# DerekRowell/AudioSDR

Hardware: AMD Instinct MI355X
Metric: Msamples/s through full SSB demod chain, batched 128-sample blocks (higher is better)
Workload: dtype f32

## Files before the change

### audiosdr_amd/csrc/asdr_kernels.hip

```cpp
#include <hip/hip_runtime.h>
#include <stdint.h>
#include <stddef.h>
#include <string.h>
#include <stdlib.h>
#include <type_traits>

#include "asdr_device.h"
#include "asdr_tables.h"
#include "../../include/asdr.h"

#define W0 0
#define W1 128
#define PH 256
#define XP 0
#ifndef ASDR_STRIDE
#define ASDR_STRIDE 388
#endif
#ifndef ASDR_AGC_QUIET_PATH
#define ASDR_AGC_QUIET_PATH 1
#endif
#ifndef ASDR_MW_OWN_STORES
#define ASDR_MW_OWN_STORES 1
#endif
#ifndef ASDR_AGC_LEAN
#define ASDR_AGC_LEAN 1
#endif
#ifndef ASDR_MW_AGC_PIPELINED
#define ASDR_MW_AGC_PIPELINED 0
#endif
#ifndef ASDR_ONEBLK
#define ASDR_ONEBLK 1
#endif
#ifndef ASDR_MW
#define ASDR_MW 1
#endif
#ifndef ASDR_MW_SHARE
#define ASDR_MW_SHARE 7
#endif
#ifndef ASDR_MIX_KEEP_Q
#define ASDR_MIX_KEEP_Q 1
#endif
#ifndef ASDR_UNIT_SCALE
#define ASDR_UNIT_SCALE 1
#endif
#ifndef ASDR_C16
#define ASDR_C16 0
#endif
#ifndef ASDR_C16_MIN_WAVES
#define ASDR_C16_MIN_WAVES 64
#endif
#ifndef ASDR_MW_MIN_WAVES
#define ASDR_MW_MIN_WAVES 64
#endif
#ifndef ASDR_MW_PRIO
#define ASDR_MW_PRIO 2
#endif
#ifndef ASDR_CHAIN_PRIO
#define ASDR_CHAIN_PRIO 0
#endif
#define CHAIN_PRIO_ON() do { if (ASDR_CHAIN_PRIO) __builtin_amdgcn_s_setprio(ASDR_CHAIN_PRIO); } while (0)
#define CHAIN_PRIO_OFF() do { if (ASDR_CHAIN_PRIO) __builtin_amdgcn_s_setprio(0); } while (0)
// ... 839 lines not shown
  constexpr bool DO1 = (ROLE == 0 || ROLE == 1 || PRE_ROLE || ROLE == 6 || ROLE == 7), DO2 = (ROLE == 0 || ROLE == 2 || POST_ROLE || ROLE == 6 || ROLE == 7),
                 DO3 = (ROLE == 0 || ROLE == 3 || POST_ROLE || ROLE == 6 || ROLE == 7);
  constexpr bool TO_ALS = (ROLE == 6 || ROLE == 7 || ROLE == 10);
#ifndef ASDR_ALS_FULL_OPT
#define ASDR_ALS_FULL_OPT 2
#endif
  constexpr bool ALS_LOOPFREE = (ASDR_ONEBLK_ALS != 0) && (ONEBLK_ || (ROLE >= 4 && !LOOPED_ROLE && ASDR_ONEBLK_ROLES));
  constexpr bool ALS_FULL_OPT = (ASDR_ALS_FULL_OPT >= 1) && ASDR_COMPACT_ROWS(STRIDE) && ALS_LOOPFREE,
                 ALS_FULL_OPT2 = (ASDR_ALS_FULL_OPT >= 2) && ASDR_COMPACT_ROWS(STRIDE) && ALS_LOOPFREE;
  constexpr bool STREAM = (ROLE >= 1 && ROLE <= 3);
  constexpr bool PIPE_PK = ((ASDR_PIPE_PK_MASK & 1) && HAS_ALS) || ((ASDR_PIPE_PK_MASK & 2) && !HAS_ALS && !HAS_SAM && ROLE == 0) ||
                           ((ASDR_PIPE_PK_MASK & 4) && (HAS_SAM || ROLE > 3)) || ((ASDR_PIPE_PK_MASK & 8) && STREAM);
  if (ROLE == 0 && a.run_if != nullptr && *a.run_if == 0u) return;
  constexpr bool MW = (WAVES > 1) && !HAS_SAM && (ROLE == 0);
  constexpr int MW_SHARE = MW ? ASDR_MW_SHARE : 0;
  const int wave = (WAVES > 1) ? (int)(threadIdx.x >> 6) : 0;
#ifndef ASDR_MW_ROT
#define ASDR_MW_ROT 0
#endif
  const uint32_t mw_b = blockIdx.x;
  const uint32_t mw_rot = (ASDR_MW_ROT == 0) ? mw_b : (ASDR_MW_ROT == 1) ? (mw_b >> 3) : (ASDR_MW_ROT == 2) ? ((mw_b >> 3) + (mw_b >> 8)) :
                          (ASDR_MW_ROT == 3) ? ((mw_b * 0x9E3779B1u) >> 30) : (ASDR_MW_ROT == 4) ? ((mw_b >> 3) % 3u) : (mw_b >> 5);
  const int mw_rel = MW ? (int)(((uint32_t)wave - mw_rot) & (uint32_t)(WAVES - 1)) : 0;
  float *const mwx = lds_wg + WAVES * 8 * STRIDE;
#ifndef ASDR_MW_STRAGGLER_PRIO
#define ASDR_MW_STRAGGLER_PRIO 0
#endif
  int *const mw_prog = reinterpret_cast<int *>(lds_wg + WAVES * 8 * STRIDE + 8 * WAVES * 16 + 260);
  int *const mw_flags = mw_prog + 4;
  constexpr bool PIPE_AGC = MW && WAVES == 4 && (MW_SHARE & 7) == 7 && (ASDR_MW_AGC_PIPELINED != 0) && (ASDR_AGC_LEAN != 0) && (ASDR_MW_OWN_STORES != 0) && ABL_ON(ABL_AGC) && ABL_ON(ABL_AF) && ABL_ON(ABL_NB);
  if constexpr (PIPE_AGC) { if (threadIdx.x < 3) mw_flags[1 + threadIdx.x] = 0; }
  if constexpr (MW && ASDR_MW_STRAGGLER_PRIO != 0) { if ((threadIdx.x & 63) == 0) mw_prog[wave] = 0; }
  auto mw_straggler = [&](int point) {
    if constexpr (MW && ASDR_MW_STRAGGLER_PRIO != 0) {
      if ((threadIdx.x & 63) == 0) mw_prog[wave] = point;
      const int4 pr = *reinterpret_cast<const int4 *>(mw_prog);
      const int behind = (pr.x < point) + (pr.y < point) + (pr.z < point) + (pr.w < point);
      const bool last = __builtin_amdgcn_readfirstlane(behind) == 0;
      if (last) __builtin_amdgcn_s_setprio(ASDR_MW_STRAGGLER_PRIO); else __builtin_amdgcn_s_setprio(0);
    }
  };
  constexpr int MWX = 16;
  auto mw_channel = [&](int q) -> int { const int sidx = (int)blockIdx.x * (8 * WAVES) + q; return (sidx < a.n_sched) ? a.direct_ch0 + sidx : a.n_channels; };
  const int wave_g = STREAM ? (int)blockIdx.x % a.stream_waves : (int)blockIdx.x * WAVES + wave;
  float *const lds = lds_wg + wave * 8 * STRIDE;
  const int lane = threadIdx.x & 63, c8 = lane >> 3, s8_ = lane & 7;
#ifndef ASDR_MW_SINE_LDS
#define ASDR_MW_SINE_LDS 0
#endif
  constexpr bool MW_SINE = MW && (ASDR_MW_SINE_LDS != 0);
  constexpr bool MW_SINE_LAZY = MW_SINE && (ASDR_MW_SINE_LDS == 2) && (MW_SHARE & 2) != 0 && WAVES == 4;
  constexpr bool SINE_LDS = HAS_SAM || (MW_SINE && !MW_SINE_LAZY);
  constexpr bool SINE_LDS_PC = HAS_SAM || MW_SINE;
  float *const sine_tab = HAS_SAM ? lds_wg + WAVES * 8 * STRIDE : (MW_SINE ? lds_wg + WAVES * 8 * STRIDE + 8 * WAVES * 16 : nullptr);
  float *const sine = SINE_LDS ? sine_tab : nullptr;
  int *const mw_sflag = reinterpret_cast<int *>(lds_wg + WAVES * 8 * STRIDE + 8 * WAVES * 16 + 260) + 8;
  if (HAS_SAM) for (int i = lane; i < ASDR_SINE_TABLE_LEN; i += 64) sine_tab[i] = c_sine[i];
  if (MW_SINE && !MW_SINE_LAZY) { for (int i = (int)threadIdx.x; i < ASDR_SINE_TABLE_LEN; i += 64 * WAVES) sine_tab[i] = c_sine[i]; __syncthreads(); }

  int4 slot = make_int4(a.n_channels, 0, 0, 0);
  const bool mw_pad = MW && (wave_g * 8 >= a.n_sched);
  if (UNIFORM && a.direct_ch0 >= 0) slot = make_int4(mw_pad ? a.n_channels : a.direct_ch0 + wave_g * 8 + c8, (int)a.direct_mode, (int)a.direct_flags, (int)((a.direct_lo & 0xFFu) | (wave_g == 0 ? a.lo_writer_bit : 0u)));
  else if (WAVES == 1 || wave_g * 8 < a.n_sched) slot = *reinterpret_cast<const int4 *>(a.sched + wave_g * 8 + c8);
  else { const ChanParams *pd = a.params + a.n_channels; slot.y = (int)pd->mode; slot.z = (int)pd->flags; }
  const int ch_ = slot.x;
  const bool valid = (UNIFORM && !mw_pad) || (ch_ < a.n_channels);
  const int loff_ = c8 * STRIDE;
#define P (*Pp)
  const ChainConsts K = a.k;

  const uint32_t mode = UNIFORM ? (uint32_t)__builtin_amdgcn_readfirstlane(slot.y) : (uint32_t)slot.y;
  const uint32_t pflags = UNIFORM ? (uint32_t)__builtin_amdgcn_readfirstlane(slot.z) : (uint32_t)slot.z;
  const uint32_t lo_slot = UNIFORM ? (uint32_t)__builtin_amdgcn_readfirstlane(slot.w) : 0u;
  const bool is_ssb = DO2 && ((mode == ASDR_USBmode) || (mode == ASDR_LSBmode) || (mode == ASDR_CW_USBmode) ||
                              (mode == ASDR_CW_LSBmode) || (mode == ASDR_WSPRmode));
#ifndef ASDR_MW_NO_AM
#define ASDR_MW_NO_AM 0
#endif
  const bool is_am = !C16 && !(MW && ASDR_MW_NO_AM) && (mode == ASDR_AMmode), is_sam = (HAS_SAM || ROLE >= 4) && (mode == ASDR_SAMmode);
// ... 65 lines not shown
#define pa_c (PLB ? (2 * (lane_i >> 4) + (lane_i & 1)) : (lane_i >> 3))
#define pa_real (PLB ? ((lane_i & 3) < 2) : ((lane_i & 7) < 4))
#if ASDR_PIPE_BANK_SELECT
#define PL_CH(c) (__builtin_amdgcn_ds_bpermute((c) << 5, ch))
#define Sp row_ptr(a.small, (uint32_t)PL_CH(pl_c) * (uint32_t)sizeof(ChanSmall))
#define Spa row_ptr(a.small, (uint32_t)PL_CH(pa_c) * (uint32_t)sizeof(ChanSmall))
#define Ppl row_ptr(a.params, (uint32_t)PL_CH(pl_c) * (uint32_t)sizeof(ChanParams))
#define Ppa row_ptr(a.params, (uint32_t)PL_CH(pa_c) * (uint32_t)sizeof(ChanParams))
#define Lp (lds + pl_c * STRIDE)
#define Lpa (lds + pa_c * STRIDE)
#else
#define PL_CH(c) ch
#define Sp S
#define Spa S
#define Ppl Pp
#define Ppa Pp
#define Lp L
#define Lpa L
#endif
    const bool af_en_pa = (PLB && !UNIFORM) ? (__builtin_amdgcn_ds_bpermute(pa_c << 5, af_en ? 1 : 0) != 0) : af_en;
    const int k0 = 16 * s8, kA = 8 * s8, kF = 4 * s8;
    const bool lead = (s8 == 0);
#ifdef ASDR_TIMELINE
    const int tl_wg = ((int)blockIdx.x == 0) ? 0 : (((int)blockIdx.x == 683) ? 1 : (((int)blockIdx.x == 1365) ? 2 : (((int)blockIdx.x == 2047) ? 3 : -1)));
    const int tl_slot = STREAM ? ((wave_g == 0) ? 2 * (3 + ROLE) + (blk & 1) : -1)
                               : (MW ? ((tl_wg < 0) ? -1 : 4 * tl_wg + wave)
                                     : ((wave_g == 0) ? 0 : ((wave_g == 2731) ? 1 : ((wave_g == 5461) ? 2 : ((wave_g == 8191) ? 3 : -1)))));
    unsigned long long *tl = reinterpret_cast<unsigned long long *>(a.taps) + 32 * (tl_slot < 0 ? 0 : tl_slot);
#define TL(i) do { if (a.taps != nullptr && tl_slot >= 0 && lane == 0) tl[i] = clock64(); } while (0)
    const bool tap_on = false;
    TL(0);
    if (MW && a.taps != nullptr && tl_slot >= 0 && lane == 0) { uint32_t hw; asm volatile("s_getreg_b32 %0, hwreg(HW_REG_HW_ID)" : "=s"(hw)); tl[29] = hw; }
#else
#define TL(i) do { } while (0)
    const bool tap_on = (a.taps != nullptr) && valid && (blk == a.n_blocks - 1);
#endif
    float *tap_base = tap_on ? a.taps + (size_t)ch * ASDR_N + kA : nullptr;
    const size_t tap_stride = (size_t)a.n_channels * ASDR_N;
#define TAP8(id, h, v) do { if (tap_on) store8(tap_base + (size_t)(id) * tap_stride + 64 * (h), v); } while (0)
#define TAP4(id, m, v) do { if (tap_on) store4(tap_base - kA + kF + (size_t)(id) * tap_stride + 32 * (m), v); } while (0)
#define TAP_ROW(id, rowoff) do { if (tap_on) { for (int h_ = 0; h_ < 2; ++h_) { float tv_[8]; load8(L + (rowoff) + kA + 64 * h_, tv_); \
                                  store8(tap_base + (size_t)(id) * tap_stride + 64 * h_, tv_); } } } while (0)

    uint32_t status = S->status;
    const uint32_t status_in = status;
    const bool mix_early = is_ssb || (DO2 && is_am);
    float mphase = 0.0f, minc = 0.0f, mphase_end = 0.0f;
    float fsh_raw = 0.0f;
    if (mix_early) {
// ... 343 lines not shown
        if (lead) *reinterpret_cast<float4 *>(mwx + MWX * (wave * 8 + c8)) = make_float4(nb_avg0, mphase, minc, __int_as_float((chain_phase_own ? 1 : 0) | ((mix_early && !lo_hit) ? 2 : 0)));
        if constexpr (PIPE_AGC) {
          if (lead) {
            const bool capable = af_en && nb_en && (!agc_en || (!is_am && agc_hc_early >= 128u && agc_hang_early >= 128u));
            const bool recent = agc_en && (agc_hang_early - agc_hc_early <= 127u);
            mwx[MWX * (wave * 8 + c8) + 7] = __int_as_float((capable ? 1 : 0) | (recent ? 2 : 0));
          }
        }
        if constexpr (MW_SINE_LAZY) {
          const uint32_t p1 = (uint32_t)__builtin_amdgcn_readfirstlane((int)__float_as_uint(mphase)), i1 = (uint32_t)__builtin_amdgcn_readfirstlane((int)__float_as_uint(minc));
          const bool differ = mix_early && !__all(__float_as_uint(mphase) == p1 && __float_as_uint(minc) == i1);
          if (lane_i == 0) mw_sflag[wave] = differ ? 1 : 0;
        }
        TL(17);
        __syncthreads();
        TL(18);
        if constexpr (MW_SINE_LAZY) {
          const int4 sf = *reinterpret_cast<const int4 *>(mw_sflag);
          if (__builtin_amdgcn_readfirstlane(sf.x | sf.y | sf.z | sf.w) != 0 && mw_rel != 0) {
#pragma unroll 1
            for (int i = (mw_rel - 1) * 64 + lane_i; i < ASDR_SINE_TABLE_LEN; i += 192) { sine_tab[i] = c_sine[i]; asm volatile("" ::: "memory"); }
          }
        }
        if (ASDR_MW_PRIO && mw_rel == 0) __builtin_amdgcn_s_setprio(ASDR_MW_PRIO);
        if (mw_rel == 0 && lane_i < 8 * WAVES) {
          const int q = lane_i;
          const float4 in4 = *reinterpret_cast<const float4 *>(mwx + MWX * q);
          const int fl = __float_as_int(in4.w);
          const bool any_phase = __any((fl & 1) != 0);
          const float pe = nb_chain(lds_wg + q * STRIDE, row_ptr(a.small, (uint32_t)mw_channel(q) * (uint32_t)sizeof(ChanSmall)), in4.x, in4.y, in4.z, any_phase, (fl & 2) != 0, nb_en, is_ssb);
          mwx[MWX * q + 4] = pe;
          if (ASDR_MW_OWN_STORES) { mwx[MWX * q] = nb_avg_end; mwx[MWX * q + 1] = __int_as_float(any_phase ? 1 : 0); }
        }
#ifndef ASDR_MW_PRIO_REL0_TAIL
#define ASDR_MW_PRIO_REL0_TAIL 0
#endif
        if (ASDR_MW_PRIO && mw_rel == 0) __builtin_amdgcn_s_setprio(ASDR_MW_PRIO_REL0_TAIL);
        TL(19);
        __syncthreads();
        TL(20);
        if constexpr (PIPE_AGC) {
          const int fl = __float_as_int(mwx[MWX * (lane_i & (8 * WAVES - 1)) + 7]);
          agc_piped = __all((fl & 1) != 0) && __any((fl & 2) != 0);
        }
        if (lead) {
          mphase_end = mwx[MWX * (wave * 8 + c8) + 4];
          if (ASDR_MW_OWN_STORES) {
            if (nb_en) S->nb_avg = mwx[MWX * (wave * 8 + c8)];
            if (mix_early && !lo_hit && __float_as_int(mwx[MWX * (wave * 8 + c8) + 1]) != 0) { if (is_ssb) S->phase_ssb = mphase_end; else S->phase_am = mphase_end; }
          }
        }
      } else {
        CHAIN_PRIO_ON();
        if (lead) mphase_end = nb_chain(L, S, nb_avg0, mphase, minc, chain_phase_own, mix_early && !lo_hit, nb_en, is_ssb);
        CHAIN_PRIO_OFF();
      }
      ph_ready = mix_early && !lo_hit;
      WAVE_SYNC();
      uint32_t fm = 0u, ft = 0u;
      if (nb_en) {
// ... 455 lines not shown
        }
#pragma unroll
        for (int j = 0; j < 4; ++j) {
          mi[j] = vi[j] * cc[j] - vq[j] * sn[j];
          mq[j] = vq[j] * cc[j] + vi[j] * sn[j];
        }
        if (qn_direct) {
#pragma unroll
          for (int j = 0; j < 4; ++j) qn[4 * m + j] = mq[j];
        } else { store4(L + W0 + kF + 32 * m, mi); store4(L + W1 + kF + 32 * m, mq); }
#ifndef ASDR_TEMPORAL_RINGS
        if (is_ssb) store4_nt(hi_ring + hs * 128 + 32 * m, mi);
#else
        if (is_ssb) store4(hi_ring + hs * 128 + 32 * m, mi);
#endif
      }
    }

    float4 af_s4 = make_float4(0.f, 0.f, 0.f, 0.f);
    float af_cf[5] = {0.f, 0.f, 0.f, 0.f, 0.f};
    float agc_gain_in = 0.f, agc_old0 = 0.f, agc_carrier0 = 0.f;
    uint32_t agc_hc0 = 0u;
    int agc_tab_idx = 0;
    const bool mw_audio_duty = (MW_SHARE & 1) && (mw_rel == 1 || mw_rel == 2);
    const int mw_casc = PLB ? (4 * (lane_i >> 4) + (lane_i & 3)) : (lane_i >> 2);
    ChanSmall *mw_af_S = S;
    auto load_af_agc_state = [&]() {
    ChanSmall *const Saf = PLB ? Spa : S; const ChanParams *const Paf = PLB ? Ppa : Pp;
    if (ABL_ON(ABL_AF) && (((MW_SHARE & 1) != 0) ? af_en : af_en_pa)) {
      if constexpr ((MW_SHARE & 1) != 0) {
        if (mw_audio_duty) {
          const int chq = mw_channel(16 * (mw_rel - 1) + mw_casc);
          mw_af_S = row_ptr(a.small, (uint32_t)chq * (uint32_t)sizeof(ChanSmall));
          af_s4 = *reinterpret_cast<const float4 *>(&mw_af_S->af_state[4 * pl_st]);
          const float *cf = &c_bq_pool[row_ptr(a.params, (uint32_t)chq * (uint32_t)sizeof(ChanParams))->audio_table][5 * pl_st];
#pragma unroll
          for (int z = 0; z < 5; ++z) af_cf[z] = cf[z];
        }
      } else {
      af_s4 = *reinterpret_cast<const float4 *>(&Saf->af_state[4 * pl_st]);
      const float *cf = &c_bq_pool[Paf->audio_table][5 * pl_st];
#pragma unroll
      for (int z = 0; z < 5; ++z) af_cf[z] = cf[z];
      }
    }
    if (ABL_ON(ABL_AGC) && agc_en) {
      agc_gain_in = S->agc_gain; agc_old0 = S->agc_old_abs; agc_hc0 = S->agc_hang_counter; agc_carrier0 = S->am_carrier;
      agc_tab_idx = P.agc_table;
    }
    };
    if constexpr (!C16) load_af_agc_state();
    TL(7);
    if (__any(is_ssb)) {
      if (is_ssb && !qn_direct) {
#pragma unroll
        for (int m = 0; m < 4; ++m) load4(L + W1 + kF + 32 * m, qn + 4 * m);
      }
      WAVE_SYNC();
      if constexpr (C16) {
#pragma unroll
        for (int m = 0; m < 4; ++m) {
#pragma unroll
          for (int j = 0; j < 4; ++j) {
            const int k = kF + 32 * m + j;
            if (k >= 1) L[XP + k - 1] = hq_o[4 * m + j];
            L[XP + 127 + k] = hq_m[4 * m + j];
            if (k < 63) L[XP + 255 + k] = qn[4 * m + j];
          }
          store4_nt(hq_ring + hs * 128 + 32 * m, qn + 4 * m);
        }
        if (lead) S->hil_slot = hs ^ 1u;
        WAVE_SYNC();
        TL(8);
        v2f fa[4], fb[4];
#pragma unroll
        for (int e = 0; e < 4; ++e) { fa[e] = (v2f){0.0f, 0.0f}; fb[e] = (v2f){0.0f, 0.0f}; }
        if (ABL_ON(ABL_HIL)) hilbert_fir<0, 4, false>(L, 4 * s8, fa);
        WAVE_SYNC();
        {
          float t[32];
#pragma unroll
          for (int q = 0; q < 8; ++q) load4(L + XP + 64 + 32 * s8 + 4 * q, t + 4 * q);
          WAVE_SYNC();
#pragma unroll
          for (int q = 0; q < 8; ++q) store4(L + XP + 32 * s8 + 4 * q, t + 4 * q);
        }
#pragma unroll
        for (int m = 0; m < 4; ++m) {
#pragma unroll
          for (int j = 0; j < 4; ++j) { const int k = kF + 32 * m + j; if (k >= 63 && k < 127) L[XP + 191 + k] = qn[4 * m + j]; }
        }
        WAVE_SYNC();
        if (ABL_ON(ABL_HIL)) hilbert_fir<0, 4, false>(L, 4 * s8, fb);
        WAVE_SYNC();
        TL(9);
        load_af_agc_state();
#pragma unroll
        for (int m = 0; m < 4; ++m) load4(hi_ring + (hs ^ 1u) * 128 + 32 * m, idl + 4 * m);
        *reinterpret_cast<float4 *>(L + W1 + 8 * s8) = make_float4(fa[0][0], fa[0][1], fa[1][0], fa[1][1]);
        *reinterpret_cast<float4 *>(L + W1 + 8 * s8 + 4) = make_float4(fa[2][0], fa[2][1], fa[3][0], fa[3][1]);
        *reinterpret_cast<float4 *>(L + W1 + 64 + 8 * s8) = make_float4(fb[0][0], fb[0][1], fb[1][0], fb[1][1]);
        *reinterpret_cast<float4 *>(L + W1 + 64 + 8 * s8 + 4) = make_float4(fb[2][0], fb[2][1], fb[3][0], fb[3][1]);
        WAVE_SYNC();
      } else {
      if (is_ssb) {
        if (!RING_PREFETCH) {
#pragma unroll
          for (int m = 0; m < 4; ++m) {
            load4(hq_ring + hs * 128 + 32 * m, hq_o + 4 * m);
            load4(hq_ring + (hs ^ 1u) * 128 + 32 * m, hq_m + 4 * m);
          }
        }
#pragma unroll
        for (int m = 0; m < 4; ++m) {
#pragma unroll
          for (int j = 0; j < 4; ++j) {
            const int k = kF + 32 * m + j;
            if (k >= 1) L[XP + k - 1] = hq_o[4 * m + j];
            L[XP + 127 + k] = hq_m[4 * m + j];
          }
        }
#pragma unroll
        for (int m = 0; m < 4; ++m) {
#pragma unroll
          for (int j = 0; j < 4; ++j) L[XP + 255 + kF + 32 * m + j] = qn[4 * m + j];
#ifndef ASDR_TEMPORAL_RINGS
          store4_nt(hq_ring + hs * 128 + 32 * m, qn + 4 * m);
#else
          store4(hq_ring + hs * 128 + 32 * m, qn + 4 * m);
#endif
        }
        if (lead) S->hil_slot = hs ^ 1u;
        carry_hs = hs ^ 1u;
      }
      WAVE_SYNC();
      TL(8);
      mw_straggler(3);
      if constexpr (R2_PREFETCH) {
        const uint32_t b2 = (uint32_t)blk + 2u;
        if (blk + 1 < a.n_blocks && (seen_in < b2 || seen_lo < b2)) {
          const uint32_t ui = (uint32_t)__builtin_amdgcn_readfirstlane((int)r2_look_in), ul = (uint32_t)__builtin_amdgcn_readfirstlane((int)r2_look_lo);
          asm volatile("" ::: "memory");
          if (ui != ASDR_STREAM_FAIL && ui > seen_in) seen_in = ui;
          if (ul != ASDR_STREAM_FAIL && ul > seen_lo) seen_lo = ul;
        }
        if (blk + 1 < a.n_blocks && seen_in != ASDR_STREAM_FAIL && seen_lo != ASDR_STREAM_FAIL && seen_in >= b2 && seen_lo >= b2) {
          const LoEntry *ln = a.lo_ring + ((blk + 1) % ASDR_LO_RING);
          const float *lp = ln->c + kF, *xp = a.xch_a + ((size_t)ch * ASDR_STREAM_DEPTH + (size_t)((blk + 1) % ASDR_STREAM_DEPTH)) * (2 * ASDR_N) + kF;
          r2n_key = ld_sc1_v4(reinterpret_cast<const float *>(ln));
#pragma unroll
          for (int m = 0; m < 4; ++m) { r2n_c4[m] = ld_sc1_v4(lp + 32 * m); r2n_s4[m] = ld_sc1_v4(lp + ASDR_N + 32 * m); r2n_vi[m] = ld_sc1_v4(xp + 32 * m); r2n_vq[m] = ld_sc1_v4(xp + ASDR_N + 32 * m); }
          r2_pref = true;
// ... 149 lines not shown
      for (int r = 0; r < 5; ++r) { const int q = s8 + 8 * r; if (q < 33) agc_t4[r] = reinterpret_cast<const float4 *>(gtab)[q]; }
      }
    }
    if constexpr ((MW_SHARE & 1) != 0) {
      if (ABL_ON(ABL_AF) && af_en) {
        if constexpr (PIPE_AGC) {
          if (agc_piped && lead && agc_en) {
            float *mq = mwx + MWX * (wave * 8 + c8);
            mq[8] = agc_old0; mq[11] = agc_al_a; mq[12] = agc_be_a;
          }
        }
        TL(21);
        if constexpr (MW && (ASDR_MW_STRAGGLER_PRIO != 0 || ASDR_MW_PRIO_REL0_TAIL != 0)) __builtin_amdgcn_s_setprio(0);
        __syncthreads();
        TL(22);
        if (mw_audio_duty) {
#ifndef ASDR_MW_PRIO_AUDIO
#define ASDR_MW_PRIO_AUDIO ASDR_MW_PRIO
#endif
          if (ASDR_MW_PRIO_AUDIO) __builtin_amdgcn_s_setprio(ASDR_MW_PRIO_AUDIO);
          const int st = pl_st;
          float sv[4];
          sv[0] = af_s4.x; sv[1] = af_s4.y; sv[2] = af_s4.z; sv[3] = af_s4.w;
          if (PIPE_AGC && agc_piped) biquad_pipe<PIPE_PK, PIPE_AGC>(lds_wg + (16 * (mw_rel - 1) + mw_casc) * STRIDE + W0, true, st, af_cf, sv, mw_flags + 1 + mw_rel, lane_i == 0);
          else biquad_pipe<PIPE_PK>(lds_wg + (16 * (mw_rel - 1) + mw_casc) * STRIDE + W0, true, st, af_cf, sv);
          *reinterpret_cast<float4 *>(&mw_af_S->af_state[4 * st]) = make_float4(sv[0], sv[1], sv[2], sv[3]);
          if (ASDR_MW_PRIO_AUDIO) __builtin_amdgcn_s_setprio(0);
        } else if constexpr (PIPE_AGC) {
          if (agc_piped) {
            if (ASDR_MW_PRIO) __builtin_amdgcn_s_setprio(ASDR_MW_PRIO);
            if (mw_rel == 0) {
              const int q = lane_i >> 1;
              float *Lc = lds_wg + q * STRIDE + 4 * (lane_i & 1);
              const float be_a = mwx[MWX * q + 12];
              const uint32_t src_lds = (uint32_t)(uintptr_t)(lds_int_ptr)(mw_flags + 2), dst_lds = (uint32_t)(uintptr_t)(lds_int_ptr)(mw_flags + 1);
              v2i pr;
              auto poll_issue = [&]() { asm volatile("ds_read_b64 %0, %1" : "=v"(pr) : "v"(src_lds) : "memory"); };
              auto poll_value = [&]() -> int {
                asm volatile("s_waitcnt lgkmcnt(0)" : "+v"(pr) :: "memory");
                return __builtin_amdgcn_readfirstlane(pr.x < pr.y ? pr.x : pr.y);
              };
              poll_issue();
              int known = poll_value();
              while (known < 1) { __builtin_amdgcn_s_sleep(2); poll_issue(); known = poll_value(); }
              float xr[4];
              load4(Lc + W0, xr);
#pragma unroll 1
              for (int c = 0; c < ASDR_N / 8; ++c) {
// ... 243 lines not shown
        if (lead) {
          const float old_end = old_end_lead;
          const float g_end = (last < 0) ? gain_in : agc_compress(tab, old_end);
          status = (status & ~ASDR_S_AGC_ACTIVE) | (((double)g_end < 0.99) ? ASDR_S_AGC_ACTIVE : 0u);
          S->agc_old_abs = old_end;
          S->agc_hang_counter = (last < 0) ? agc_hc0 - 128u : agc_hang - (uint32_t)(127 - last);
          S->agc_gain = g_end;
        }
      };
      if constexpr ((MW_SHARE & 4) != 0) {
        constexpr bool LEAN_OK = (ASDR_AGC_LEAN != 0) && (ASDR_MW_OWN_STORES != 0);
        if (!agc_piped) {
        if (lead) {
          float *mq = mwx + MWX * (wave * 8 + c8);
          mq[5] = __int_as_float(agc_quiet ? 1 : 0); mq[6] = am_clamped;
          if (ASDR_MW_OWN_STORES && !agc_quiet) {
            *reinterpret_cast<float4 *>(mq + 8) = make_float4(agc_old0, __uint_as_float(agc_hc0), gain_in, agc_al_a);
            *reinterpret_cast<float4 *>(mq + 12) = make_float4(agc_be_a, agc_al_r, agc_be_r, __uint_as_float(agc_hang));
          }
        }
        TL(25);
        __syncthreads();
        TL(26);
        if (ASDR_MW_PRIO && mw_rel == 3) __builtin_amdgcn_s_setprio(ASDR_MW_PRIO);
        if (mw_rel == 3 && lane_i < 8 * WAVES) {
          const int q = lane_i;
          const bool active = (__float_as_int(mwx[MWX * q + 5]) == 0);
          float4 i0 = make_float4(0.f, 0.f, 0.f, 0.f), i1 = i0;
          if (ASDR_MW_OWN_STORES && active) { i0 = *reinterpret_cast<const float4 *>(mwx + MWX * q + 8); i1 = *reinterpret_cast<const float4 *>(mwx + MWX * q + 12); }
          const bool lean = LEAN_OK && !is_am && __all(!active || (__float_as_uint(i0.y) >= 128u && __float_as_uint(i1.w) >= 128u));
          if (q == 0) mw_flags[0] = lean ? 1 : 0;
          if (lean) {
            if (active) {
              float *Lc = lds_wg + q * STRIDE;
              float old_abs = i0.x;
              const float al_a = i0.w, be_a = i1.x;
              float x_[8];
              load8(Lc + AGC_GV, x_);
#pragma unroll 1
              for (int i2 = 0; i2 < ASDR_N; i2 += 16) {
                float xn_[8];
#pragma unroll
                for (int half = 0; half < 2; ++half) {
                  const int i = i2 + 8 * half;
                  float *x = half ? xn_ : x_, *xn = half ? x_ : xn_;
                  load8(Lc + AGC_GV + ((i + 8 < ASDR_N) ? i + 8 : i), xn);
                  float pb[8], ov[8];
#pragma unroll
// ... 4 lines not shown
                    const float v_new = pa + pb[u];
                    old_abs = (x[u] > old_abs) ? v_new : old_abs;
                    ov[u] = old_abs;
                  }
                  store8(Lc + AGC_GV + i, ov);
                }
              }
              mwx[MWX * q + 8] = old_abs;
            }
          } else
          if (active) {
            if (ASDR_MW_OWN_STORES) {
              mwx[MWX * q + 7] = agc_chain(std::true_type{}, lds_wg + q * STRIDE, nullptr, i0.x, __float_as_uint(i0.y), i0.z, i0.w, i1.x, i1.y, i1.z, __float_as_uint(i1.w), is_am, mwx[MWX * q + 6]);
              mwx[MWX * q + 8] = agc_old_end; mwx[MWX * q + 9] = __uint_as_float(agc_hc_end);
            } else {
            const int chq = mw_channel(q);
            ChanSmall *Sq = row_ptr(a.small, (uint32_t)chq * (uint32_t)sizeof(ChanSmall));
            const ChanParams *Pq = row_ptr(a.params, (uint32_t)chq * (uint32_t)sizeof(ChanParams));
            mwx[MWX * q + 7] = agc_chain(std::false_type{}, lds_wg + q * STRIDE, Sq, Sq->agc_old_abs, Sq->agc_hang_counter, Sq->agc_gain, Pq->agc_alpha_att, Pq->agc_beta_att,
                                       Pq->agc_alpha_rel, Pq->agc_beta_rel, Pq->agc_hang_count, is_am, mwx[MWX * q + 6]);
            }
          }
        }
        if (ASDR_MW_PRIO && mw_rel == 3) __builtin_amdgcn_s_setprio(0);
        TL(27);
        __syncthreads();
        TL(28);
        } else { TL(25); TL(26); TL(27); TL(28); }
        const bool lean_done = LEAN_OK && (agc_piped || __builtin_amdgcn_readfirstlane(mw_flags[0]) != 0);
        if (lean_done && !agc_quiet && agc_en) {
          agc_lean_finish(lead ? mwx[MWX * (wave * 8 + c8) + 8] : 0.0f);
        } else
        if (!agc_quiet && lead) {
          const float *mq = mwx + MWX * (wave * 8 + c8);
          const float g_end = mq[7]; status = (status & ~ASDR_S_AGC_ACTIVE) | (((double)g_end < 0.99) ? ASDR_S_AGC_ACTIVE : 0u);
          if (ASDR_MW_OWN_STORES && agc_en) { S->agc_old_abs = mq[8]; S->agc_hang_counter = __float_as_uint(mq[9]); S->agc_gain = g_end; }
        }
      } else {
#ifndef ASDR_AGC_LEAN1
#define ASDR_AGC_LEAN1 1
#endif
        constexpr bool LEAN1_OK = (ASDR_AGC_LEAN1 != 0) && !C16 && !(ROLE == 0 && WAVES == 1 && !ONEBLK_ && !HAS_ALS && !HAS_SAM && UNIFORM);
        const bool lean1 = LEAN1_OK && !agc_quiet && __all(!(agc_en && lead) || (!is_am && agc_hc0 >= 128u && agc_hang >= 128u));
        if (!agc_quiet) CHAIN_PRIO_ON();
        if (lean1) {
          float old_abs = agc_old0;
          if (agc_en && lead) {
// ... 219 lines not shown
#undef pl_st
#undef pl_iq
#undef pl_c
#undef pa_c
#undef pa_real
}

#define ASDR_KERNEL(name, lds_floats, bounds, stride, als, sam, uni, waves)                                     \
  extern "C" __global__ __launch_bounds__(64 * waves, bounds) void name(UpdateArgs a) {                         \
    __shared__ __attribute__((aligned(16))) float lds[lds_floats];                                              \
    asdr_update_body<stride, als, sam, uni, waves>(a, lds);                                                     \
  }
ASDR_KERNEL(asdr_update_kernel, 8 * ASDR_STRIDE, ASDR_WAVES_PER_EU, ASDR_STRIDE, false, false, true, 1)
ASDR_KERNEL(asdr_update_kernel_mixed, 8 * ASDR_STRIDE, ASDR_WAVES_PER_EU, ASDR_STRIDE, false, false, false, 1)
extern "C" __global__ __launch_bounds__(64, ASDR_WAVES_PER_EU) void asdr_update_kernel_one(UpdateArgs a) {
  __shared__ __attribute__((aligned(16))) float lds[8 * ASDR_STRIDE];
  asdr_update_body<ASDR_STRIDE, false, false, true, 1, 0, true>(a, lds);
}
#define ASDR_C16_STRIDE 320
extern "C" __global__ __launch_bounds__(64, 4) void asdr_update_kernel_c16(UpdateArgs a) {
  __shared__ __attribute__((aligned(16))) float lds[8 * ASDR_C16_STRIDE];
  asdr_update_body<ASDR_C16_STRIDE, false, false, true, 1, 0, true>(a, lds);
}
#define ASDR_MW_WAVES 4
extern "C" __global__ __launch_bounds__(64 * ASDR_MW_WAVES, ASDR_WAVES_PER_EU) void asdr_update_kernel_mw(UpdateArgs a) {
  __shared__ __attribute__((aligned(16))) float lds[ASDR_MW_WAVES * 8 * ASDR_STRIDE + ASDR_MW_WAVES * 8 * 16 + 260 + 12];
  asdr_update_body<ASDR_STRIDE, false, false, true, ASDR_MW_WAVES, 0, true>(a, lds);
}
ASDR_KERNEL(asdr_update_kernel_sam, ASDR_SAM_WAVES * 8 * ASDR_STRIDE + 260, ASDR_WAVES_PER_EU, ASDR_STRIDE, false, true, false, ASDR_SAM_WAVES)
#ifndef ASDR_ALS_WAVES_PER_EU
#define ASDR_ALS_WAVES_PER_EU 3
#endif
#ifndef ASDR_ALS_LDS_PAD
#define ASDR_ALS_LDS_PAD 0
#endif
ASDR_KERNEL(asdr_update_kernel_als, 8 * 516 + 260 + ASDR_ALS_LDS_PAD, ASDR_ALS_WAVES_PER_EU, 516, true, true, true, 1)
ASDR_KERNEL(asdr_update_kernel_als_mixed, 8 * 516 + 260 + ASDR_ALS_LDS_PAD, ASDR_ALS_WAVES_PER_EU, 516, true, true, false, 1)
ASDR_KERNEL(asdr_update_kernel_als_small, 8 * ASDR_ALS_STRIDE, ASDR_WAVES_PER_EU, ASDR_ALS_STRIDE, true, false, true, 1)
ASDR_KERNEL(asdr_update_kernel_als_small_mixed, 8 * ASDR_ALS_STRIDE, ASDR_WAVES_PER_EU, ASDR_ALS_STRIDE, true, false, false, 1)
extern "C" __global__ __launch_bounds__(64, ASDR_WAVES_PER_EU) void asdr_update_kernel_als_small_one(UpdateArgs a) {
  __shared__ __attribute__((aligned(16))) float lds[8 * ASDR_ALS_STRIDE];
  asdr_update_body<ASDR_ALS_STRIDE, true, false, true, 1, 0, true>(a, lds);
}

extern "C" __global__ __launch_bounds__(64, ASDR_WAVES_PER_EU) void asdr_sam_pre_kernel(UpdateArgs a) {
  __shared__ __attribute__((aligned(16))) float lds[8 * ASDR_STRIDE];
  asdr_update_body<ASDR_STRIDE, false, false, false, 1, 4>(a, lds);
}
extern "C" __global__ __launch_bounds__(64, ASDR_WAVES_PER_EU) void asdr_sam_post_kernel(UpdateArgs a) {
  __shared__ __attribute__((aligned(16))) float lds[8 * ASDR_STRIDE];
// ... 279 lines not shown
  "asdr_sam_post_als_kernel",
  "asdr_sam_post_als_kernel_uniform",
  "asdr_sam_post_kernel",
  "asdr_sam_post_kernel_uniform",
  "asdr_sam_post_loop_kernel_uniform",
  "asdr_sam_pre_kernel",
  "asdr_sam_pre_kernel_uniform",
  "asdr_sam_pre_loop_kernel_uniform",
  "asdr_spin_kernel",
  "asdr_stream_ack_kernel",
  "asdr_stream_kernel",
  "asdr_stream_kernel_h3",
  "asdr_stream_restore_kernel",
  "asdr_stream_snapshot_kernel",
  "asdr_update_kernel",
  "asdr_update_kernel_als",
  "asdr_update_kernel_als_mixed",
  "asdr_update_kernel_als_small",
  "asdr_update_kernel_als_small_mixed",
  "asdr_update_kernel_als_small_one",
  "asdr_update_kernel_c16",
  "asdr_update_kernel_mixed",
  "asdr_update_kernel_mw",
  "asdr_update_kernel_one",
  "asdr_update_kernel_sam"
};
#define ASDR_N_KERNEL_NAMES ((int)(sizeof k_kernel_names / sizeof k_kernel_names[0]))
static unsigned long long g_kernel_launches[ASDR_N_KERNEL_NAMES];
static inline int kernel_name_index(const char *name) {
  for (int i = 0; i < ASDR_N_KERNEL_NAMES; ++i)
    if (strcmp(k_kernel_names[i], name) == 0) return i;
  return -1;
}
static inline void count_launch(int i) { if (i >= 0) __atomic_fetch_add(&g_kernel_launches[i], 1ull, __ATOMIC_RELAXED); }
#define ASDR_LAUNCH(kernel, ...) do { static const int site_index_ = kernel_name_index(#kernel); count_launch(site_index_); hipLaunchKernelGGL(kernel, __VA_ARGS__); } while (0)
extern "C" int asdr_kernels_count(void) { return ASDR_N_KERNEL_NAMES; }
extern "C" const char *asdr_kernels_name(int i) { return (i >= 0 && i < ASDR_N_KERNEL_NAMES) ? k_kernel_names[i] : nullptr; }
extern "C" unsigned long long asdr_kernels_launches(int i) { return (i >= 0 && i < ASDR_N_KERNEL_NAMES) ? __atomic_load_n(&g_kernel_launches[i], __ATOMIC_RELAXED) : 0ull; }
extern "C" void asdr_kernels_launches_reset(void) { for (int i = 0; i < ASDR_N_KERNEL_NAMES; ++i) __atomic_store_n(&g_kernel_launches[i], 0ull, __ATOMIC_RELAXED); }

extern "C" int asdr_launch_stream(const UpdateArgs *a, hipStream_t stream, int fir_helpers) {
  if (a->stream_waves <= 0) return 0;
  if (fir_helpers == 3) ASDR_LAUNCH(asdr_stream_kernel_h3, dim3(3 * a->stream_waves), dim3(256), 0, stream, *a);
  else ASDR_LAUNCH(asdr_stream_kernel, dim3(3 * a->stream_waves), dim3(128), 0, stream, *a);
  return hipGetLastError() == hipSuccess ? 0 : -1;
}
// ... 81 lines not shown
extern "C" int asdr_launch_update(const UpdateArgs *a, int variant, int uniform, hipStream_t stream) {
  const int n_waves = a->n_sched / 8;
  if (n_waves <= 0) return 0;
  if (variant == ASDR_KERNEL_ALS || (variant == ASDR_KERNEL_SAM_ALS && a->xch_sam == nullptr)) { if (uniform) ASDR_LAUNCH(asdr_update_kernel_als, dim3(n_waves), dim3(64), 0, stream, *a); else ASDR_LAUNCH(asdr_update_kernel_als_mixed, dim3(n_waves), dim3(64), 0, stream, *a); }
  else if (variant == ASDR_KERNEL_ALS_SMALL && uniform == 2) {
    ASDR_LAUNCH(asdr_als_pre_kernel, dim3(n_waves), dim3(64), 0, stream, *a);
    ASDR_LAUNCH(asdr_als_kernel, dim3(n_waves), dim3(64), 0, stream, *a);
  }
  else if (variant == ASDR_KERNEL_ALS_SMALL) { if (uniform && ASDR_ONEBLK && ASDR_ONEBLK_ALS && a->n_blocks == 1 && a->run_if == nullptr) ASDR_LAUNCH(asdr_update_kernel_als_small_one, dim3(n_waves), dim3(64), 0, stream, *a); else if (uniform) ASDR_LAUNCH(asdr_update_kernel_als_small, dim3(n_waves), dim3(64), 0, stream, *a); else ASDR_LAUNCH(asdr_update_kernel_als_small_mixed, dim3(n_waves), dim3(64), 0, stream, *a); }
  else if ((variant == ASDR_KERNEL_SAM || variant == ASDR_KERNEL_SAM_ALS) && a->xch_sam != nullptr) {
    if (uniform) ASDR_LAUNCH(asdr_sam_pre_kernel_uniform, dim3(n_waves), dim3(64), 0, stream, *a);
    else ASDR_LAUNCH(asdr_sam_pre_kernel, dim3(n_waves), dim3(64), 0, stream, *a);
    ASDR_LAUNCH(asdr_sam_pll_kernel, dim3((a->n_sched + ASDR_PLL_LANES - 1) / ASDR_PLL_LANES), dim3(64), 0, stream, *a);
    if (variant == ASDR_KERNEL_SAM_ALS) {
      if (uniform) ASDR_LAUNCH(asdr_sam_post_als_kernel_uniform, dim3(n_waves), dim3(64), 0, stream, *a);
      else ASDR_LAUNCH(asdr_sam_post_als_kernel, dim3(n_waves), dim3(64), 0, stream, *a);
    } else {
      if (uniform) ASDR_LAUNCH(asdr_sam_post_kernel_uniform, dim3(n_waves), dim3(64), 0, stream, *a);
      else ASDR_LAUNCH(asdr_sam_post_kernel, dim3(n_waves), dim3(64), 0, stream, *a);
    }
  }
  else if (variant == ASDR_KERNEL_SAM) ASDR_LAUNCH(asdr_update_kernel_sam, dim3((n_waves + ASDR_SAM_WAVES - 1) / ASDR_SAM_WAVES), dim3(64 * ASDR_SAM_WAVES), 0, stream, *a);
  else {
    static int mw_on = -1, mw_min = ASDR_MW_MIN_WAVES, c16_on = ASDR_C16, c16_min = ASDR_C16_MIN_WAVES, c16_pad = 0;
    if (mw_on < 0) {
      const char *e = getenv("ASDR_MW"); mw_on = e ? atoi(e) : ASDR_MW; const char *m = getenv("ASDR_MW_MIN_WAVES"); if (m) mw_min = atoi(m);
      const char *c = getenv("ASDR_C16"); if (c) c16_on = atoi(c); const char *cm = getenv("ASDR_C16_MIN_WAVES"); if (cm) c16_min = atoi(cm);
      const char *cp = getenv("ASDR_C16_PAD"); if (cp) c16_pad = atoi(cp);
    }
    const uint32_t dm = a->direct_mode;
    const bool ssb_class = dm == ASDR_USBmode || dm == ASDR_LSBmode || dm == ASDR_CW_USBmode || dm == ASDR_CW_LSBmode || dm == ASDR_WSPRmode;
    if (uniform && c16_on && a->n_blocks == 1 && a->run_if == nullptr && a->direct_ch0 >= 0 && a->taps == nullptr && ssb_class && n_waves >= c16_min)
      ASDR_LAUNCH(asdr_update_kernel_c16, dim3(n_waves), dim3(64), (size_t)c16_pad, stream, *a);
    else
    if (uniform && mw_on && a->n_blocks == 1 && a->run_if == nullptr && a->direct_ch0 >= 0 && n_waves >= mw_min)
      ASDR_LAUNCH(asdr_update_kernel_mw, dim3((n_waves + ASDR_MW_WAVES - 1) / ASDR_MW_WAVES), dim3(64 * ASDR_MW_WAVES), 0, stream, *a);
    else
    if (uniform && ASDR_ONEBLK && a->n_blocks == 1 && a->run_if == nullptr) ASDR_LAUNCH(asdr_update_kernel_one, dim3(n_waves), dim3(64), 0, stream, *a);
    else if (uniform) ASDR_LAUNCH(asdr_update_kernel, dim3(n_waves), dim3(64), 0, stream, *a);
    else ASDR_LAUNCH(asdr_update_kernel_mixed, dim3(n_waves), dim3(64), 0, stream, *a);
  }
  return hipGetLastError() == hipSuccess ? 0 : -1;
}

extern "C" __global__ void asdr_als_stage_seed_kernel(UpdateArgs a, int ch0, int n) {
  const int c = (int)blockIdx.x, t = (int)threadIdx.x;
  if (c >= n) return;
  const size_t ch = (size_t)(ch0 + c);
  a.als_stage[ch * (ASDR_ALS_STAGE_SLOTS * ASDR_N) + a.als_stage_prev * ASDR_N + t] = a.als_x[ch * (2 * ASDR_N) + ((a.als_phase & 1u) ^ 1u) * ASDR_N + t];
}
extern "C" int asdr_launch_als_role(const UpdateArgs *a, int role, hipStream_t stream) {
  const int n_waves = a->n_sched / 8;
  if (n_waves <= 0) return 0;
  if (role == 2) ASDR_LAUNCH(asdr_sam_pre_loop_kernel_uniform, dim3(n_waves), dim3(64), 0, stream, *a);
  else if (role == 3) ASDR_LAUNCH(asdr_als_back_loop_kernel, dim3(n_waves), dim3(64), 0, stream, *a);
  else if (role == 0 && a->n_blocks > 1) ASDR_LAUNCH(asdr_als_pre_loop_kernel, dim3(n_waves), dim3(64), 0, stream, *a);
  else if (role == 0) ASDR_LAUNCH(asdr_als_pre_kernel, dim3(n_waves), dim3(64), 0, stream, *a);
  else ASDR_LAUNCH(asdr_als_kernel, dim3(n_waves), dim3(64), 0, stream, *a);
  return hipGetLastError() == hipSuccess ? 0 : -1;
// ... 46 lines not shown
```

Baseline: 81660.

## Add two-wave MW kernel variant, shrink MW LDS, vectorize Hilbert ring stores

Adds an asdr_update_kernel_mw2 variant that runs the multi-wave path with two waves per workgroup, remapping the shared NB, audio and AGC duties for that size. The variant is selectable through the ASDR_MW_WAVES environment variable and defaults to four waves. When the MW sine table is disabled, its 260 floats of LDS are no longer reserved, which may raise occupancy. The Hilbert quadrature window layout is also shifted by one element so its LDS stores become aligned float4 stores instead of scalar stores, with a cross-lane ds_bpermute supplying the shifted neighbour value.

```diff
diff --git a/audiosdr_amd/csrc/asdr_kernels.hip b/audiosdr_amd/csrc/asdr_kernels.hip
--- a/audiosdr_amd/csrc/asdr_kernels.hip
+++ b/audiosdr_amd/csrc/asdr_kernels.hip
@@ -37,6 +37,10 @@
 #ifndef ASDR_MW_SHARE
 #define ASDR_MW_SHARE 7
 #endif
+#ifndef ASDR_MW_SINE_LDS
+#define ASDR_MW_SINE_LDS 0
+#endif
+#define ASDR_MW_SINE_FLOATS ((ASDR_MW_SINE_LDS != 0) ? 260 : 0)
 #ifndef ASDR_MIX_KEEP_Q
 #define ASDR_MIX_KEEP_Q 1
 #endif
@@ -922,11 +926,15 @@
   const uint32_t mw_rot = (ASDR_MW_ROT == 0) ? mw_b : (ASDR_MW_ROT == 1) ? (mw_b >> 3) : (ASDR_MW_ROT == 2) ? ((mw_b >> 3) + (mw_b >> 8)) :
                           (ASDR_MW_ROT == 3) ? ((mw_b * 0x9E3779B1u) >> 30) : (ASDR_MW_ROT == 4) ? ((mw_b >> 3) % 3u) : (mw_b >> 5);
   const int mw_rel = MW ? (int)(((uint32_t)wave - mw_rot) & (uint32_t)(WAVES - 1)) : 0;
+  static_assert(!MW || WAVES == 2 || WAVES == 4, "the shared duties are laid out for workgroups of two or four waves");
+  constexpr int MW_REL_NB = (WAVES == 2) ? 1 : 0, MW_REL_AGC = (WAVES == 2) ? 1 : 3;
+  const bool mw_rel_audio = (WAVES == 2) ? (mw_rel == 0) : (mw_rel == 1 || mw_rel == 2);
+  const int mw_audio_q0 = (WAVES == 2) ? 0 : 16 * (mw_rel - 1);
   float *const mwx = lds_wg + WAVES * 8 * STRIDE;
 #ifndef ASDR_MW_STRAGGLER_PRIO
 #define ASDR_MW_STRAGGLER_PRIO 0
 #endif
-  int *const mw_prog = reinterpret_cast<int *>(lds_wg + WAVES * 8 * STRIDE + 8 * WAVES * 16 + 260);
+  int *const mw_prog = reinterpret_cast<int *>(lds_wg + WAVES * 8 * STRIDE + 8 * WAVES * 16 + ASDR_MW_SINE_FLOATS);
   int *const mw_flags = mw_prog + 4;
   constexpr bool PIPE_AGC = MW && WAVES == 4 && (MW_SHARE & 7) == 7 && (ASDR_MW_AGC_PIPELINED != 0) && (ASDR_AGC_LEAN != 0) && (ASDR_MW_OWN_STORES != 0) && ABL_ON(ABL_AGC) && ABL_ON(ABL_AF) && ABL_ON(ABL_NB);
   if constexpr (PIPE_AGC) { if (threadIdx.x < 3) mw_flags[1 + threadIdx.x] = 0; }
@@ -954,7 +962,7 @@
   constexpr bool SINE_LDS_PC = HAS_SAM || MW_SINE;
   float *const sine_tab = HAS_SAM ? lds_wg + WAVES * 8 * STRIDE : (MW_SINE ? lds_wg + WAVES * 8 * STRIDE + 8 * WAVES * 16 : nullptr);
   float *const sine = SINE_LDS ? sine_tab : nullptr;
-  int *const mw_sflag = reinterpret_cast<int *>(lds_wg + WAVES * 8 * STRIDE + 8 * WAVES * 16 + 260) + 8;
+  int *const mw_sflag = reinterpret_cast<int *>(lds_wg + WAVES * 8 * STRIDE + 8 * WAVES * 16 + ASDR_MW_SINE_FLOATS) + 8;
   if (HAS_SAM) for (int i = lane; i < ASDR_SINE_TABLE_LEN; i += 64) sine_tab[i] = c_sine[i];
   if (MW_SINE && !MW_SINE_LAZY) { for (int i = (int)threadIdx.x; i < ASDR_SINE_TABLE_LEN; i += 64 * WAVES) sine_tab[i] = c_sine[i]; __syncthreads(); }
 
@@ -1066,9 +1074,10 @@
     const int k0 = 16 * s8, kA = 8 * s8, kF = 4 * s8;
     const bool lead = (s8 == 0);
 #ifdef ASDR_TIMELINE
-    const int tl_wg = ((int)blockIdx.x == 0) ? 0 : (((int)blockIdx.x == 683) ? 1 : (((int)blockIdx.x == 1365) ? 2 : (((int)blockIdx.x == 2047) ? 3 : -1)));
+    constexpr int TL_WGS = MW ? 4 / WAVES : 1;
+    const int tl_wg = ((int)blockIdx.x == 0) ? 0 : (((int)blockIdx.x == 683 * TL_WGS) ? 1 : (((int)blockIdx.x == 1365 * TL_WGS) ? 2 : (((int)blockIdx.x == 2047 * TL_WGS) ? 3 : -1)));
     const int tl_slot = STREAM ? ((wave_g == 0) ? 2 * (3 + ROLE) + (blk & 1) : -1)
-                               : (MW ? ((tl_wg < 0) ? -1 : 4 * tl_wg + wave)
+                               : (MW ? ((tl_wg < 0) ? -1 : WAVES * tl_wg + wave)
                                      : ((wave_g == 0) ? 0 : ((wave_g == 2731) ? 1 : ((wave_g == 5461) ? 2 : ((wave_g == 8191) ? 3 : -1)))));
     unsigned long long *tl = reinterpret_cast<unsigned long long *>(a.taps) + 32 * (tl_slot < 0 ? 0 : tl_slot);
 #define TL(i) do { if (a.taps != nullptr && tl_slot >= 0 && lane == 0) tl[i] = clock64(); } while (0)
@@ -1458,8 +1467,8 @@
             for (int i = (mw_rel - 1) * 64 + lane_i; i < ASDR_SINE_TABLE_LEN; i += 192) { sine_tab[i] = c_sine[i]; asm volatile("" ::: "memory"); }
           }
         }
-        if (ASDR_MW_PRIO && mw_rel == 0) __builtin_amdgcn_s_setprio(ASDR_MW_PRIO);
-        if (mw_rel == 0 && lane_i < 8 * WAVES) {
+        if (ASDR_MW_PRIO && mw_rel == MW_REL_NB) __builtin_amdgcn_s_setprio(ASDR_MW_PRIO);
+        if (mw_rel == MW_REL_NB && lane_i < 8 * WAVES) {
           const int q = lane_i;
           const float4 in4 = *reinterpret_cast<const float4 *>(mwx + MWX * q);
           const int fl = __float_as_int(in4.w);
@@ -1471,7 +1480,7 @@
 #ifndef ASDR_MW_PRIO_REL0_TAIL
 #define ASDR_MW_PRIO_REL0_TAIL 0
 #endif
-        if (ASDR_MW_PRIO && mw_rel == 0) __builtin_amdgcn_s_setprio(ASDR_MW_PRIO_REL0_TAIL);
+        if (ASDR_MW_PRIO && mw_rel == MW_REL_NB) __builtin_amdgcn_s_setprio(ASDR_MW_PRIO_REL0_TAIL);
         TL(19);
         __syncthreads();
         TL(20);
@@ -1973,7 +1982,7 @@
     float agc_gain_in = 0.f, agc_old0 = 0.f, agc_carrier0 = 0.f;
     uint32_t agc_hc0 = 0u;
     int agc_tab_idx = 0;
-    const bool mw_audio_duty = (MW_SHARE & 1) && (mw_rel == 1 || mw_rel == 2);
+    const bool mw_audio_duty = (MW_SHARE & 1) && mw_rel_audio;
     const int mw_casc = PLB ? (4 * (lane_i >> 4) + (lane_i & 3)) : (lane_i >> 2);
     ChanSmall *mw_af_S = S;
     auto load_af_agc_state = [&]() {
@@ -1981,7 +1990,7 @@
     if (ABL_ON(ABL_AF) && (((MW_SHARE & 1) != 0) ? af_en : af_en_pa)) {
       if constexpr ((MW_SHARE & 1) != 0) {
         if (mw_audio_duty) {
-          const int chq = mw_channel(16 * (mw_rel - 1) + mw_casc);
+          const int chq = mw_channel(mw_audio_q0 + mw_casc);
           mw_af_S = row_ptr(a.small, (uint32_t)chq * (uint32_t)sizeof(ChanSmall));
           af_s4 = *reinterpret_cast<const float4 *>(&mw_af_S->af_state[4 * pl_st]);
           const float *cf = &c_bq_pool[row_ptr(a.params, (uint32_t)chq * (uint32_t)sizeof(ChanParams))->audio_table][5 * pl_st];
@@ -2008,17 +2017,29 @@
         for (int m = 0; m < 4; ++m) load4(L + W1 + kF + 32 * m, qn + 4 * m);
       }
       WAVE_SYNC();
+      auto hq_next = [&](int m) -> float {
+        const int src = ((s8 == 7) ? lane_i - 7 : lane_i + 1) << 2;
+        return __int_as_float(__builtin_amdgcn_ds_bpermute(src, __float_as_int((s8 == 0) ? qn[4 * ((m + 1) & 3)] : qn[4 * m])));
+      };
+      auto hq_window_ends = [&](float next3) {
+        hq_o[15] = (s8 == 7) ? hq_m[15] : hq_o[15];
+        hq_m[15] = (s8 == 7) ? next3 : hq_m[15];
+      };
       if constexpr (C16) {
+        float qr[16];
+#pragma unroll
+        for (int m = 0; m < 4; ++m) { qr[4 * m] = qn[4 * m + 1]; qr[4 * m + 1] = qn[4 * m + 2]; qr[4 * m + 2] = qn[4 * m + 3]; qr[4 * m + 3] = hq_next(m); }
+        hq_window_ends(qr[15]);
 #pragma unroll
         for (int m = 0; m < 4; ++m) {
+          store4(L + XP + kF + 32 * m, hq_o + 4 * m);
+          store4(L + XP + 128 + kF + 32 * m, hq_m + 4 * m);
 #pragma unroll
           for (int j = 0; j < 4; ++j) {
-            const int k = kF + 32 * m + j;
-            if (k >= 1) L[XP + k - 1] = hq_o[4 * m + j];
-            L[XP + 127 + k] = hq_m[4 * m + j];
-            if (k < 63) L[XP + 255 + k] = qn[4 * m + j];
-          }
-          store4_nt(hq_ring + hs * 128 + 32 * m, qn + 4 * m);
+            const int w = kF + 32 * m + j;
+            if (w < 62) L[XP + 256 + w] = qr[4 * m + j];
+          }
+          store4_nt(hq_ring + hs * 128 + 32 * m, qr + 4 * m);
         }
         if (lead) S->hil_slot = hs ^ 1u;
         WAVE_SYNC();
@@ -2039,7 +2060,7 @@
 #pragma unroll
         for (int m = 0; m < 4; ++m) {
 #pragma unroll
-          for (int j = 0; j < 4; ++j) { const int k = kF + 32 * m + j; if (k >= 63 && k < 127) L[XP + 191 + k] = qn[4 * m + j]; }
+          for (int j = 0; j < 4; ++j) { const int w = kF + 32 * m + j; if (w >= 62 && w < 126) L[XP + 192 + w] = qr[4 * m + j]; }
         }
         WAVE_SYNC();
         if (ABL_ON(ABL_HIL)) hilbert_fir<0, 4, false>(L, 4 * s8, fb);
@@ -2062,23 +2083,21 @@
             load4(hq_ring + (hs ^ 1u) * 128 + 32 * m, hq_m + 4 * m);
           }
         }
+        hq_window_ends(hq_next(3));
 #pragma unroll
         for (int m = 0; m < 4; ++m) {
-#pragma unroll
-          for (int j = 0; j < 4; ++j) {
-            const int k = kF + 32 * m + j;
-            if (k >= 1) L[XP + k - 1] = hq_o[4 * m + j];
-            L[XP + 127 + k] = hq_m[4 * m + j];
-          }
+          store4(L + XP + kF + 32 * m, hq_o + 4 * m);
+          store4(L + XP + 128 + kF + 32 * m, hq_m + 4 * m);
         }
 #pragma unroll
         for (int m = 0; m < 4; ++m) {
-#pragma unroll
-          for (int j = 0; j < 4; ++j) L[XP + 255 + kF + 32 * m + j] = qn[4 * m + j];
+          const float qr[4] = {qn[4 * m + 1], qn[4 * m + 2], qn[4 * m + 3], hq_next(m)};
+          if (m < 3 || s8 < 7) store4(L + XP + 256 + kF + 32 * m, qr);
+          else { L[XP + 380] = qr[0]; L[XP + 381] = qr[1]; L[XP + 382] = qr[2]; }
 #ifndef ASDR_TEMPORAL_RINGS
-          store4_nt(hq_ring + hs * 128 + 32 * m, qn + 4 * m);
+          store4_nt(hq_ring + hs * 128 + 32 * m, qr);
 #else
-          store4(hq_ring + hs * 128 + 32 * m, qn + 4 * m);
+          store4(hq_ring + hs * 128 + 32 * m, qr);
 #endif
         }
         if (lead) S->hil_slot = hs ^ 1u;
@@ -2274,8 +2293,8 @@
           const int st = pl_st;
           float sv[4];
           sv[0] = af_s4.x; sv[1] = af_s4.y; sv[2] = af_s4.z; sv[3] = af_s4.w;
-          if (PIPE_AGC && agc_piped) biquad_pipe<PIPE_PK, PIPE_AGC>(lds_wg + (16 * (mw_rel - 1) + mw_casc) * STRIDE + W0, true, st, af_cf, sv, mw_flags + 1 + mw_rel, lane_i == 0);
-          else biquad_pipe<PIPE_PK>(lds_wg + (16 * (mw_rel - 1) + mw_casc) * STRIDE + W0, true, st, af_cf, sv);
+          if (PIPE_AGC && agc_piped) biquad_pipe<PIPE_PK, PIPE_AGC>(lds_wg + (mw_audio_q0 + mw_casc) * STRIDE + W0, true, st, af_cf, sv, mw_flags + 1 + mw_rel, lane_i == 0);
+          else biquad_pipe<PIPE_PK>(lds_wg + (mw_audio_q0 + mw_casc) * STRIDE + W0, true, st, af_cf, sv);
           *reinterpret_cast<float4 *>(&mw_af_S->af_state[4 * st]) = make_float4(sv[0], sv[1], sv[2], sv[3]);
           if (ASDR_MW_PRIO_AUDIO) __builtin_amdgcn_s_setprio(0);
         } else if constexpr (PIPE_AGC) {
@@ -2565,8 +2584,8 @@
         TL(25);
         __syncthreads();
         TL(26);
-        if (ASDR_MW_PRIO && mw_rel == 3) __builtin_amdgcn_s_setprio(ASDR_MW_PRIO);
-        if (mw_rel == 3 && lane_i < 8 * WAVES) {
+        if (ASDR_MW_PRIO && mw_rel == MW_REL_AGC) __builtin_amdgcn_s_setprio(ASDR_MW_PRIO);
+        if (mw_rel == MW_REL_AGC && lane_i < 8 * WAVES) {
           const int q = lane_i;
           const bool active = (__float_as_int(mwx[MWX * q + 5]) == 0);
           float4 i0 = make_float4(0.f, 0.f, 0.f, 0.f), i1 = i0;
@@ -2617,7 +2636,7 @@
             }
           }
         }
-        if (ASDR_MW_PRIO && mw_rel == 3) __builtin_amdgcn_s_setprio(0);
+        if (ASDR_MW_PRIO && mw_rel == MW_REL_AGC) __builtin_amdgcn_s_setprio(0);
         TL(27);
         __syncthreads();
         TL(28);
@@ -2883,10 +2902,17 @@
   __shared__ __attribute__((aligned(16))) float lds[8 * ASDR_C16_STRIDE];
   asdr_update_body<ASDR_C16_STRIDE, false, false, true, 1, 0, true>(a, lds);
 }
+#define ASDR_MW_LDS_FLOATS(waves) ((waves) * 8 * ASDR_STRIDE + (waves) * 8 * 16 + ASDR_MW_SINE_FLOATS + 12)
+extern "C" __global__ __launch_bounds__(64 * 4, ASDR_WAVES_PER_EU) void asdr_update_kernel_mw(UpdateArgs a) {
+  __shared__ __attribute__((aligned(16))) float lds[ASDR_MW_LDS_FLOATS(4)];
+  asdr_update_body<ASDR_STRIDE, false, false, true, 4, 0, true>(a, lds);
+}
+#ifndef ASDR_MW_WAVES
 #define ASDR_MW_WAVES 4
-extern "C" __global__ __launch_bounds__(64 * ASDR_MW_WAVES, ASDR_WAVES_PER_EU) void asdr_update_kernel_mw(UpdateArgs a) {
-  __shared__ __attribute__((aligned(16))) float lds[ASDR_MW_WAVES * 8 * ASDR_STRIDE + ASDR_MW_WAVES * 8 * 16 + 260 + 12];
-  asdr_update_body<ASDR_STRIDE, false, false, true, ASDR_MW_WAVES, 0, true>(a, lds);
+#endif
+extern "C" __global__ __launch_bounds__(64 * 2, ASDR_WAVES_PER_EU) void asdr_update_kernel_mw2(UpdateArgs a) {
+  __shared__ __attribute__((aligned(16))) float lds[ASDR_MW_LDS_FLOATS(2)];
+  asdr_update_body<ASDR_STRIDE, false, false, true, 2, 0, true>(a, lds);
 }
 ASDR_KERNEL(asdr_update_kernel_sam, ASDR_SAM_WAVES * 8 * ASDR_STRIDE + 260, ASDR_WAVES_PER_EU, ASDR_STRIDE, false, true, false, ASDR_SAM_WAVES)
 #ifndef ASDR_ALS_WAVES_PER_EU
@@ -3212,6 +3238,7 @@
   "asdr_update_kernel_c16",
   "asdr_update_kernel_mixed",
   "asdr_update_kernel_mw",
+  "asdr_update_kernel_mw2",
   "asdr_update_kernel_one",
   "asdr_update_kernel_sam"
 };
@@ -3339,9 +3366,10 @@
   }
   else if (variant == ASDR_KERNEL_SAM) ASDR_LAUNCH(asdr_update_kernel_sam, dim3((n_waves + ASDR_SAM_WAVES - 1) / ASDR_SAM_WAVES), dim3(64 * ASDR_SAM_WAVES), 0, stream, *a);
   else {
-    static int mw_on = -1, mw_min = ASDR_MW_MIN_WAVES, c16_on = ASDR_C16, c16_min = ASDR_C16_MIN_WAVES, c16_pad = 0;
+    static int mw_on = -1, mw_min = ASDR_MW_MIN_WAVES, mw_waves = ASDR_MW_WAVES, c16_on = ASDR_C16, c16_min = ASDR_C16_MIN_WAVES, c16_pad = 0;
     if (mw_on < 0) {
       const char *e = getenv("ASDR_MW"); mw_on = e ? atoi(e) : ASDR_MW; const char *m = getenv("ASDR_MW_MIN_WAVES"); if (m) mw_min = atoi(m);
+      const char *w = getenv("ASDR_MW_WAVES"); if (w) mw_waves = atoi(w);
       const char *c = getenv("ASDR_C16"); if (c) c16_on = atoi(c); const char *cm = getenv("ASDR_C16_MIN_WAVES"); if (cm) c16_min = atoi(cm);
       const char *cp = getenv("ASDR_C16_PAD"); if (cp) c16_pad = atoi(cp);
     }
@@ -3350,8 +3378,10 @@
     if (uniform && c16_on && a->n_blocks == 1 && a->run_if == nullptr && a->direct_ch0 >= 0 && a->taps == nullptr && ssb_class && n_waves >= c16_min)
       ASDR_LAUNCH(asdr_update_kernel_c16, dim3(n_waves), dim3(64), (size_t)c16_pad, stream, *a);
     else
-    if (uniform && mw_on && a->n_blocks == 1 && a->run_if == nullptr && a->direct_ch0 >= 0 && n_waves >= mw_min)
-      ASDR_LAUNCH(asdr_update_kernel_mw, dim3((n_waves + ASDR_MW_WAVES - 1) / ASDR_MW_WAVES), dim3(64 * ASDR_MW_WAVES), 0, stream, *a);
+    if (uniform && mw_on && a->n_blocks == 1 && a->run_if == nullptr && a->direct_ch0 >= 0 && n_waves >= mw_min) {
+      if (mw_waves == 2) ASDR_LAUNCH(asdr_update_kernel_mw2, dim3((n_waves + 1) / 2), dim3(64 * 2), 0, stream, *a);
+      else ASDR_LAUNCH(asdr_update_kernel_mw, dim3((n_waves + 3) / 4), dim3(64 * 4), 0, stream, *a);
+    }
     else
     if (uniform && ASDR_ONEBLK && a->n_blocks == 1 && a->run_if == nullptr) ASDR_LAUNCH(asdr_update_kernel_one, dim3(n_waves), dim3(64), 0, stream, *a);
     else if (uniform) ASDR_LAUNCH(asdr_update_kernel, dim3(n_waves), dim3(64), 0, stream, *a);
```

After: 82010 (median of 6 runs). Within noise of the previous version (+0.4%).
